# FifthEpoch/longcat-video-tta

Hardware: AMD Instinct MI355X
Metric: denoised latent frames/sec (49x720p, 50-step CFG denoise) (higher is better)
Workload: dtype bf16; 1 GPU; K3: 49x720p (13 latent frames, 46 800 tokens); DiT 48 blocks x 4096 hidden, CFG 4.0, 50-step flow-match Euler, no conditioning frames; depth=48, parallelism=dp1

## Files before the change

### longcat-video-tta_amd/csrc/attn_fwd.hip

```cpp
#include "attn_common.h"
#include <type_traits>

struct AttnFwdParams : AttnFwdLead {
  float scale, scale_log2e;
  int gx, xcd_remap;
};

template <int NWAVES, int PRIO, bool XATTN, int VAR>
__global__ __launch_bounds__(NWAVES * 64) void attn_fwd_kernel(const AttnFwdParams p) {
  constexpr bool DMA = (VAR & 1) != 0;
  constexpr bool UNIT = (VAR & 2) != 0;
  static_assert(!DMA || NWAVES == 8, "LDS-DMA staging is laid out for 8 waves (2 K + 2 V instructions per wave)");
  constexpr int NT = NWAVES * 64;
  constexpr int QROWS = NWAVES * 32;
  constexpr int NCH = 1024 / NT;
  constexpr int TILE_BYTES = 64 * 256;
  extern __shared__ __attribute__((aligned(16))) unsigned char smem[];
  lds_u8* lds = (lds_u8*)smem;

  const int tid = threadIdx.x;
  const int lane = tid & 63;
  const int wave = __builtin_amdgcn_readfirstlane(tid >> 6);
  const int r = lane & 31, h = lane >> 5;
  int qb, head;
// ... 102 lines not shown
  if (PRIO == 1 && wave >= NWAVES / 2) __builtin_amdgcn_s_setprio(1);
  const int nt = (int)((p.d.Nk + 63) / 64);
  {
    if (DMA) {
      dma_tile(0, 0, std::false_type{});
    } else {
      load_tile(0);
      store_tile(0);
    }
    __syncthreads();
  }

  auto tile_body = [&](const int t, auto buf_c, auto last_c, auto next_full_c) {
    constexpr int buf = decltype(buf_c)::value;
    constexpr bool has_next = !decltype(last_c)::value;
    if (has_next) {
      if (DMA) dma_tile(t + 1, buf ^ 1, next_full_c);
      else load_tile((int64_t)(t + 1) * 64);
    }

    const lds_u8* kb = lds + buf * 2 * TILE_BYTES;
    const lds_u8* vb = kb + TILE_BYTES;

    f32x16 s0, s1;
#pragma unroll
    for (int e = 0; e < 16; ++e) { s0[e] = UNIT ? minit[e] : 0.f; s1[e] = UNIT ? minit[e] : 0.f; }
#pragma unroll
    for (int ks = 0; ks < 8; ++ks) {
      const int co = 16 * ((2 * ks + h) ^ kf);
      const bf16x8 a0 = *reinterpret_cast<const __attribute__((address_space(3))) bf16x8*>(kb + k_row_off + co);
      const bf16x8 a1 = *reinterpret_cast<const __attribute__((address_space(3))) bf16x8*>(kb + 32 * 256 + k_row_off + co);
      s0 = __builtin_amdgcn_mfma_f32_32x32x16_bf16(a0, qf[ks], s0, 0, 0, 0);
      s1 = __builtin_amdgcn_mfma_f32_32x32x16_bf16(a1, qf[ks], s1, 0, 0, 0);
    }

    if (!has_next && (p.d.Nk & 63)) {
      const int valid = (int)(p.d.Nk - (int64_t)t * 64);
#pragma unroll
      for (int e = 0; e < 16; ++e) {
        const int key = (e & 3) + 8 * (e >> 2) + 4 * h;
        if (key >= valid) s0[e] = -INFINITY;
        if (key + 32 >= valid) s1[e] = -INFINITY;
      }
    }

    float mxa = s0[0], mxb = s1[0];
#pragma unroll
    for (int e = 1; e < 16; ++e) {
      mxa = fmaxf(mxa, s0[e]);
      mxb = fmaxf(mxb, s1[e]);
    }
    float mx = fmaxf(mxa, mxb);
    mx = half_max(mx);
    float psum = 0.f;
    if constexpr (UNIT) {
      if (__builtin_amdgcn_ballot_w64(mx > ATTN_RESCALE_THR) != 0ull || t == 0) {
        const float d = (t == 0) ? mx : fmaxf(mx, 0.f);
        const float alpha = __builtin_amdgcn_exp2f(-d);
        m_run += d;
        l_run *= alpha;
#pragma unroll
        for (int dd = 0; dd < 4; ++dd)
#pragma unroll
          for (int e = 0; e < 16; ++e) oacc[dd][e] *= alpha;
#pragma unroll
        for (int e = 0; e < 16; ++e) {
          s0[e] -= d;
          s1[e] -= d;
          minit[e] = -m_run;
        }
      }
#pragma unroll
      for (int e = 0; e < 16; ++e) {
        s0[e] = __builtin_amdgcn_exp2f(s0[e]);
        s1[e] = __builtin_amdgcn_exp2f(s1[e]);
        psum += s0[e] + s1[e];
      }
    } else {
      if (__builtin_amdgcn_ballot_w64((mx - m_run) * p.scale_log2e > ATTN_RESCALE_THR) != 0ull) {
        const float m_new = fmaxf(m_run, mx);
        const float alpha = __builtin_amdgcn_exp2f((m_run - m_new) * p.scale_log2e);
        m_run = m_new;
        l_run *= alpha;
#pragma unroll
        for (int d = 0; d < 4; ++d)
#pragma unroll
          for (int e = 0; e < 16; ++e) oacc[d][e] *= alpha;
      }
      const float mc = m_run * p.scale_log2e;
#pragma unroll
      for (int e = 0; e < 16; ++e) {
        s0[e] = __builtin_amdgcn_exp2f(s0[e] * p.scale_log2e - mc);
        s1[e] = __builtin_amdgcn_exp2f(s1[e] * p.scale_log2e - mc);
        psum += s0[e] + s1[e];
      }
    }
    l_run += psum;

    bf16x8 pb[4];
#pragma unroll
    for (int j = 0; j < 8; ++j) {
      pb[0][j] = (__bf16)s0[j];
      pb[1][j] = (__bf16)s0[8 + j];
      pb[2][j] = (__bf16)s1[j];
      pb[3][j] = (__bf16)s1[8 + j];
    }

#pragma unroll
    for (int kk = 0; kk < 4; ++kk) {
#pragma unroll
      for (int d = 0; d < 4; ++d) {
        const int dx = 64 * (d ^ q4);
        const s16x4 lo = __builtin_amdgcn_ds_read_tr16_b64_v4i16(
            (__attribute__((address_space(3))) s16x4*)(vb + v_base[0] + 4096 * kk + dx + 16 * v_low[0]));
        const s16x4 hi = __builtin_amdgcn_ds_read_tr16_b64_v4i16(
            (__attribute__((address_space(3))) s16x4*)(vb + v_base[1] + 4096 * kk + dx + 16 * v_low[1]));
        const bf16x8 vf = __builtin_bit_cast(bf16x8, __builtin_shufflevector(lo, hi, 0, 1, 2, 3, 4, 5, 6, 7));
        oacc[d] = __builtin_amdgcn_mfma_f32_32x32x16_bf16(vf, pb[kk], oacc[d], 0, 0, 0);
      }
    }

    if (has_next && !DMA) store_tile(buf ^ 1);
    __syncthreads();
  };
  {
    using B0 = std::integral_constant<int, 0>;
    using B1 = std::integral_constant<int, 1>;
    using Y = std::true_type;
    using N = std::false_type;
    int t = 0;
    for (; t + 3 < nt; t += 2) {
      tile_body(t, B0{}, N{}, Y{});
      tile_body(t + 1, B1{}, N{}, Y{});
    }
    const int left = nt - t;
    if (left == 3) {
      tile_body(t, B0{}, N{}, Y{});
      tile_body(t + 1, B1{}, N{}, N{});
      tile_body(t + 2, B0{}, Y{}, N{});
    } else if (left == 2) {
      tile_body(t, B0{}, N{}, N{});
      tile_body(t + 1, B1{}, Y{}, N{});
    } else {
      tile_body(t, B0{}, Y{}, N{});
    }
  }

  const float l_tot = half_sum(l_run);
  const float inv = 1.0f / l_tot;
  const int64_t qrow = q0 + r;
  if (qrow < p.d.Nq) {
    bf16_t* op = p.o + b * p.d.o_sb + qrow * p.d.o_sn + (int64_t)head * p.d.o_sh;
#pragma unroll
    for (int d = 0; d < 4; ++d)
#pragma unroll
      for (int i = 0; i < 4; ++i) {
        u16x4 pk;
#pragma unroll
        for (int e = 0; e < 4; ++e) pk[e] = f2bf(oacc[d][4 * i + e] * inv);
        *reinterpret_cast<u16x4*>(op + 32 * d + 8 * i + 4 * h) = pk;
      }
    if (p.lse && h == 0) p.lse[(b * p.d.H + head) * p.d.Nq + qrow] = m_run * p.scale + __logf(l_tot);
  }
}

static thread_local const char* g_last_attn_kernel = "none";
extern "C" const char* lcv_attn_fwd_last_kernel(void) { return g_last_attn_kernel; }

extern "C" int lcv_attn_fwd(const void* q, const void* k, const void* v, void* o, float* lse, int64_t B,
                            int64_t H, int64_t Nq, int64_t Nk, int64_t q_sb, int64_t q_sn, int64_t q_sh,
                            int64_t k_sb, int64_t k_sn, int64_t k_sh, int64_t v_sb, int64_t v_sn,
                            int64_t v_sh, int64_t o_sb, int64_t o_sn, int64_t o_sh, float scale,
                            void* stream) {
  LCV_CHECK_ARG(q && k && v && o, "attn_fwd: null pointer");
  LCV_CHECK_ARG(B > 0 && H > 0 && H <= 65535 && B <= 65535, "attn_fwd: bad B/H");
  LCV_CHECK_ARG(Nk > 0, "attn_fwd: Nk must be > 0 (empty key set has no softmax)");
  LCV_CHECK_ARG(q_sn % 8 == 0 && k_sn % 8 == 0 && v_sn % 8 == 0 && q_sh % 8 == 0 && k_sh % 8 == 0 &&
                    v_sh % 8 == 0 && q_sb % 8 == 0 && k_sb % 8 == 0 && v_sb % 8 == 0,
                "attn_fwd: q/k/v strides must be multiples of 8 elements");
  LCV_CHECK_ARG(o_sn % 4 == 0 && o_sh % 4 == 0 && o_sb % 4 == 0, "attn_fwd: o strides must be multiples of 4 elements");
  LCV_CHECK_ARG(((uintptr_t)q % 16 == 0) && ((uintptr_t)k % 16 == 0) && ((uintptr_t)v % 16 == 0) && ((uintptr_t)o % 8 == 0),
                "attn_fwd: pointers must be 16-byte aligned");
  if (Nq == 0) return LCV_OK;
  AttnArgs a = {};
// ... 38 lines not shown
```

### longcat-video-tta_amd/csrc/elementwise.hip

```cpp
#include "lcv_common.h"
#include "cfg_guidance.h"

#define ROWNORM_MAXCH 8

template <int MODE>
__global__ __launch_bounds__(256) void rownorm_fwd_kernel(
    const bf16_t* __restrict__ x, const float* __restrict__ p_add, const float* __restrict__ p_mul,
    bf16_t* __restrict__ y, int64_t rows, int C, int64_t S, int64_t mod_stride, float eps) {
  const int lane = threadIdx.x & 63;
  const int64_t row = (int64_t)blockIdx.x * 4 + (threadIdx.x >> 6);
  if (row >= rows) return;
  const bf16_t* xr = x + row * C;
  float v[ROWNORM_MAXCH][8];
  float sum = 0.f;
#pragma unroll
  for (int ch = 0; ch < ROWNORM_MAXCH; ++ch) {
    const int c = (ch * 64 + lane) * 8;
    if (c < C) {
      u16x8 raw = *reinterpret_cast<const u16x8*>(xr + c);
      unpack8(raw, v[ch]);
#pragma unroll
      for (int i = 0; i < 8; ++i) sum += v[ch][i];
    } else {
#pragma unroll
// ... 96 lines not shown
}

extern "C" int lcv_gate_residual_fwd(const void* x, const void* y, const float* mod, void* out,
                                     int64_t B, int64_t T, int64_t S, int64_t C, int64_t mod_stride,
                                     int64_t gate_off, void* stream) {
  LCV_CHECK_ARG(x && y && out, "gate_residual_fwd: null pointer");
  LCV_CHECK_ARG(C > 0 && C % 8 == 0, "gate_residual_fwd: C must be a multiple of 8");
  LCV_CHECK_ARG(gate_off % 4 == 0 && mod_stride % 4 == 0, "gate_residual_fwd: offsets must be 16-byte aligned");
  const int64_t n_packets = B * T * S * (C / 8);
  if (n_packets == 0) return LCV_OK;
  int64_t blocks = (n_packets + 255) / 256;
  if (blocks > 256 * 16) blocks = 256 * 16;
  hipLaunchKernelGGL(gate_residual_fwd_kernel, dim3((unsigned)blocks), dim3(256), 0, (hipStream_t)stream,
                     (const bf16_t*)x, (const bf16_t*)y, mod ? mod + gate_off : nullptr, (bf16_t*)out,
                     n_packets, (int)(C / 8), S, mod_stride);
  LCV_LAUNCH_CHECK("gate_residual_fwd");
  return LCV_OK;
}

__device__ __forceinline__ void norm_rope_vec(const bf16_t* src, bf16_t* dst, const float (&w)[8],
                                              const float (&cs)[8], bool do_rope, float eps, float out_scale) {
  float f[8];
  unpack8(*reinterpret_cast<const u16x8*>(src), f);
  float ss = 0.f;
#pragma unroll
  for (int i = 0; i < 8; ++i) ss += f[i] * f[i];
  ss += __shfl_xor(ss, 8, 64);
  ss += __shfl_xor(ss, 4, 64);
  ss += __shfl_xor(ss, 2, 64);
  ss += __shfl_xor(ss, 1, 64);
  const float r = rsqrtf(ss * (1.0f / 128.0f) + eps);
  float o[8];
#pragma unroll
  for (int i = 0; i < 8; ++i) f[i] = bfround(bfround(f[i] * r) * w[i]);
  if (do_rope) {
#pragma unroll
    for (int i = 0; i < 4; ++i) {
      const float c = cs[2 * i], s = cs[2 * i + 1];
      const float x0 = f[2 * i], x1 = f[2 * i + 1];
      o[2 * i] = __fadd_rn(__fmul_rn(x0, c), __fmul_rn(-x1, s));
      o[2 * i + 1] = __fadd_rn(__fmul_rn(x1, c), __fmul_rn(x0, s));
    }
  } else {
#pragma unroll
    for (int i = 0; i < 8; ++i) o[i] = f[i];
  }
#pragma unroll
  for (int i = 0; i < 8; ++i) o[i] *= out_scale;
  *reinterpret_cast<u16x8*>(dst) = pack8(o);
}

__global__ __launch_bounds__(256) void qknorm_rope_fwd_kernel(
    const bf16_t* __restrict__ q_in, const bf16_t* __restrict__ k_in, const bf16_t* __restrict__ v_in,
    bf16_t* __restrict__ q_out, bf16_t* __restrict__ k_out, bf16_t* __restrict__ v_out,
    const bf16_t* __restrict__ wq, const bf16_t* __restrict__ wk, const float* __restrict__ cs_tab,
    int H, int64_t in_sb, int64_t in_sn, int64_t q_sb, int64_t q_sn, int64_t kv_sb, int64_t kv_sn,
    int64_t pos_off, float eps, float q_scale) {
// ... 398 lines not shown
```

### longcat-video-tta_amd/lcv_hip/autograd_ops.py

```python
import weakref
from typing import List, Optional

import torch

from . import ops
from .lib import (LCV_EPI_GELU_TANH, LCV_EPI_NONE, LCV_EPI_SWIGLU, LcvError)

BF16 = torch.bfloat16
F32 = torch.float32

_EPI = {None: LCV_EPI_NONE, "gelu_tanh": LCV_EPI_GELU_TANH}


def _needs_grad(*ts) -> bool:
    return torch.is_grad_enabled() and any(t is not None and t.requires_grad for t in ts)


_WT_CACHE = {}


def transposed_weight(w: torch.Tensor) -> torch.Tensor:
    key = id(w)
    ent = _WT_CACHE.get(key)
    if ent is not None and ent[0]() is w and ent[1] == w._version and ent[2].data_ptr() != 0:
# ... 467 lines not shown
        off = 0
        for b in range(B):
            Lb = int(seqlens[b])
            ops.attention_bwd(qn[b:b + 1], kn[:, off:off + Lb], kv_raw[:, off:off + Lb, 1], o[b:b + 1], do[b:b + 1],
                              lses[b], dqn[b:b + 1], dkv[:, off:off + Lb, 0], dkv[:, off:off + Lb, 1], scale,
                              accumulate_kv=False)
            off += Lb
        dq_raw = torch.empty_like(q_raw)
        dwq = torch.zeros(D, dtype=torch.float32, device=q_raw.device) if want_dw else None
        dwk = torch.zeros(D, dtype=torch.float32, device=q_raw.device) if want_dw else None
        ops.qknorm_rope_bwd(q_raw, None, dqn, None, dq_raw, None, wq, wk, None, 0, eps, dwq=dwq)
        dkv_raw = torch.empty_like(kv_raw)
        ops.qknorm_rope_bwd(None, kv_raw[:, :, 0], None, dkv[:, :, 0], None, dkv_raw[:, :, 0], wq, wk, None, 0, eps, dwk=dwk)
        dkv_raw[:, :, 1].copy_(dkv[:, :, 1])
        return (dq_raw, dkv_raw, dwq.to(wq.dtype) if (want_dw and wq.requires_grad) else None,
                dwk.to(wk.dtype) if (want_dw and wk.requires_grad) else None, None, None, None)


def cross_attention(q, kv, wq, wk, seqlens: List[int], scale, eps):
    if _needs_grad(q, kv, wq, wk):
        return _CrossAttentionFn.apply(q, kv, wq, wk, seqlens, scale, eps)
    B, N, H, D = q.shape
    k, v = kv[:, :, 0], kv[:, :, 1]
    ops.qknorm_rope(q, None, None, q, None, None, wq, wk, None, 0, eps)
    ops.qknorm_rope(None, k, None, None, k, None, wq, wk, None, 0, eps)
    o = torch.empty_like(q)
    off = 0
    for b in range(B):
        Lb = int(seqlens[b])
        ops.attention(q[b:b + 1], k[:, off:off + Lb], v[:, off:off + Lb], scale, out=o[b:b + 1])
        off += Lb
    return o


class _GeluTanhFn(torch.autograd.Function):
    @staticmethod
    def forward(ctx, x):
        ctx.save_for_backward(x)
        return ops.gelu_tanh(x)

    @staticmethod
    def backward(ctx, dy):
        (x,) = ctx.saved_tensors
        return ops.gelu_tanh_bwd(x, (dy if dy.dtype == BF16 else dy.to(BF16)).contiguous())


def gelu_tanh(x: torch.Tensor) -> torch.Tensor:
    if _needs_grad(x):
        return _GeluTanhFn.apply(x)
# ... 105 lines not shown
```

### longcat-video-tta_amd/lcv_hip/build.py

```python
import os
import subprocess
import sys
from concurrent.futures import ThreadPoolExecutor
from pathlib import Path

PKG_DIR = Path(__file__).resolve().parent
CSRC = PKG_DIR.parent / "csrc"
INCLUDE = PKG_DIR.parents[1] / "include"
BUILD = CSRC / "build"
LIB = PKG_DIR / "liblcv_hip.so"
HIPCC = os.environ.get("HIPCC", "/opt/rocm/bin/hipcc")
FLAGS = ["--offload-arch=gfx950", "-O3", "-fPIC", "-std=c++17", "-Wno-unused-value",
         "-fno-gpu-rdc", "-I", str(INCLUDE)]


def _newest_header():
    hs = list(CSRC.glob("*.h")) + list(INCLUDE.glob("*.h"))
    return max(h.stat().st_mtime for h in hs)


_ATTN_FLAGS = ["-fno-honor-nans", "-mno-amdgpu-ieee", "-fno-slp-vectorize"]
EXTRA = {"attn_fwd.hip": _ATTN_FLAGS, "attn_fwd_pipe.hip": _ATTN_FLAGS, "attn_bwd_dq2.hip": _ATTN_FLAGS, "attn_bwd_dkv2.hip": _ATTN_FLAGS,
         "attn_fwd_w64.hip": _ATTN_FLAGS,
         "optim_master.hip": ["-ffp-contract=off"], "optim_moments8.hip": ["-ffp-contract=off"],
         "optim_accum.hip": ["-ffp-contract=off"], "optim_anchor.hip": ["-ffp-contract=off"],
         "optim_ema.hip": ["-ffp-contract=off"], "step_cache.hip": ["-ffp-contract=off"],
         "solver_step.hip": ["-ffp-contract=off"], "cfg_reuse.hip": ["-ffp-contract=off"]}


def _compile(src: Path, hdr_mtime: float) -> Path:
    obj = BUILD / (src.stem + ".o")
    if obj.exists() and obj.stat().st_mtime > max(src.stat().st_mtime, hdr_mtime):
        return obj
    cmd = [HIPCC, *FLAGS, *EXTRA.get(src.name, []), "-c", str(src), "-o", str(obj)]
    r = subprocess.run(cmd, capture_output=True, text=True)
    if r.returncode != 0:
        raise RuntimeError(f"hipcc failed for {src.name}:\n{r.stdout}\n{r.stderr}")
    if r.stderr.strip():
        sys.stderr.write(r.stderr)
    return obj


def build(verbose: bool = False) -> Path:
    BUILD.mkdir(exist_ok=True)
    srcs = sorted(CSRC.glob("*.hip"))
    if not srcs:
# ... 18 lines not shown
```

### longcat-video-tta_amd/lcv_hip/lib.py

```python
import ctypes
import os
from ctypes import c_char_p, c_double, c_float, c_int, c_int64, c_uint64, c_void_p
from pathlib import Path

_LIB_PATH = Path(__file__).resolve().parent / "liblcv_hip.so"

P, I64, F32, I, F64, U64 = c_void_p, c_int64, c_float, c_int, c_double, c_uint64

_SIGNATURES = {
    "lcv_device_check": [],
    "lcv_adaln_modulate_fwd": [P, P, P, I64, I64, I64, I64, I64, I64, I64, F32, P],
    "lcv_adaln_modulate_bwd": [P, P, P, P, P, I64, I64, I64, I64, I64, I64, I64, F32, P, P],
    "lcv_layernorm_affine_fwd": [P, P, P, P, I64, I64, F32, P],
    "lcv_layernorm_affine_bwd": [P, P, P, P, P, P, I64, I64, F32, P, P],
    "lcv_gate_residual_fwd": [P, P, P, P, I64, I64, I64, I64, I64, I64, P],
    "lcv_gate_residual_bwd": [P, P, P, P, P, I64, I64, I64, I64, I64, I64, P],
    "lcv_qknorm_rope_fwd": [P, P, P, P, P, P, P, P, P, I64, I64, I64, I64, I64, I64, I64, I64, I64, I64, F32, F32, P],
    "lcv_qknorm_rope_bwd": [P, P, P, P, P, P, P, P, P, I64, I64, I64, I64, I64, I64, I64, I64, I64, I64, I64, I64, F32, F32, P, P, I64, P],
    "lcv_attn_fwd": [P, P, P, P, P, I64, I64, I64, I64] + [I64] * 12 + [F32, P],
    "lcv_attn_bwd": [P, P, P, P, P, P, P, P, P, P, I, I64, I64, I64, I64] + [I64] * 21 + [F32, P],
    "lcv_gemm_nt": [P, P, P, P, P, P, I64, I64, I64, I64, I64, I64, I64, I64, I64, I, I, P, P, I64, I64, I64, P],
    "lcv_gemm_set_workspace": [P, I64],
    "lcv_linear_f32_smallm": [P, P, P, P, I64, I64, I64, I, P],
    "lcv_lora_down": [P, P, P, I64, I64, I64, I64, I64, F32, P],
# ... 84 lines not shown
}

_SIGNATURES_EMA = {
    "lcv_master_ema_load": [P, P, P, I64, I64, P],
    "lcv_master_ema_update": [P, P, P, I64, I64, F64, P],
    "lcv_master_ema_swap": [P, P, P, I64, I64, P],
}

_SIGNATURES_STEPCACHE = {
    "lcv_stepcache_diff": [P, P, P, P, I64, I64, F32, P, I64, P, P],
    "lcv_stepcache_store": [P, P, P, I64, P],
    "lcv_stepcache_apply": [P, P, P, I64, P],
}

_SIGNATURES_SOLVER = {
    "lcv_cfg_lms_step": [P, P, P, P, P, P, P, I64, I64, F32, F32, F32, F32, I, I, I, P],
}

_SIGNATURES_CFGREUSE = {
    "lcv_cfg_delta_store": [P, P, P, P, P, I64, I64, F32, I, P],
    "lcv_cfg_delta_apply": [P, P, P, I64, I64, P],
}

LCV_EPI_NONE, LCV_EPI_SWIGLU, LCV_EPI_GATE_RESIDUAL, LCV_EPI_GELU_TANH, LCV_EPI_SILU = 0, 1, 2, 3, 4


class LcvError(RuntimeError):
    code = None

    @property
    def fatal(self) -> bool:
        return self.code in (-2, -3)


_lib = None


def lib_path() -> Path:
    return _LIB_PATH


def load():
    global _lib
    if _lib is not None:
        return _lib
    if not _LIB_PATH.exists():
# ... 8 lines not shown
    lib.lcv_last_error.argtypes = []
    lib.lcv_attn_fwd_last_kernel.restype = c_char_p
    lib.lcv_attn_fwd_last_kernel.argtypes = []
    lib.lcv_knobs_list.restype = c_char_p
    lib.lcv_knobs_list.argtypes = []
    lib.lcv_knobs_reload.restype = c_int
    lib.lcv_knobs_reload.argtypes = []
    lib.lcv_conv3d_last_kernel.restype = c_char_p
    lib.lcv_conv3d_last_kernel.argtypes = []
    lib.lcv_tn_skinny_ws_bytes.restype = c_int64
    lib.lcv_tn_skinny_ws_bytes.argtypes = [I64, I64, I64]
    lib.lcv_attn_bwd_ws_floats.restype = c_int64
    lib.lcv_attn_bwd_ws_floats.argtypes = [I64, I64, I64, I64]
    lib.lcv_lpips_ws_bytes.restype = c_int64
    lib.lcv_lpips_ws_bytes.argtypes = [I64, I64, I64]
    lib.lcv_det_ws_bytes.restype = c_int64
    lib.lcv_det_ws_bytes.argtypes = [I, I64, I64, I64]
    lib.lcv_tn_skinny_dropout_ws_bytes.restype = c_int64
    lib.lcv_tn_skinny_dropout_ws_bytes.argtypes = [I64, I64, I64]
    for name, args in (list(_SIGNATURES.items()) + list(_SIGNATURES_LPIPS.items()) + list(_SIGNATURES_DET.items())
                       + list(_SIGNATURES_LORA.items()) + list(_SIGNATURES_MASTER.items()) + list(_SIGNATURES_MOMENTS8.items())
                       + list(_SIGNATURES_ACCUM.items()) + list(_SIGNATURES_ANCHOR.items()) + list(_SIGNATURES_EMA.items())
                       + list(_SIGNATURES_STEPCACHE.items()) + list(_SIGNATURES_SOLVER.items())
                       + list(_SIGNATURES_CFGREUSE.items())):
        fn = getattr(lib, name, None)
        if fn is None:
            continue
        fn.restype = c_int
        fn.argtypes = args
    _lib = lib
    return lib


def reload_knobs() -> int:
    return load().lcv_knobs_reload()


def set_knob(name: str, value) -> None:
    if value is None:
        os.environ.pop(name, None)
    else:
        os.environ[name] = str(value)
    if _lib is not None:
        _lib.lcv_knobs_reload()


def call(name: str, *args):
# ... 9 lines not shown
```

### longcat-video-tta_amd/lcv_hip/ops.py

```python
import os
from typing import Optional, Tuple

import torch

from . import lib as _lib
from .lib import (LCV_EPI_GATE_RESIDUAL, LCV_EPI_GELU_TANH, LCV_EPI_NONE, LCV_EPI_SILU, LCV_EPI_SWIGLU,
                  call)

BF16 = torch.bfloat16
F32 = torch.float32
PROFILE = None
PROFILE_BWD = None


_DETERMINISTIC = os.environ.get("LCV_DETERMINISTIC", "") == "1"


def set_deterministic(flag: bool) -> None:
    global _DETERMINISTIC
    _DETERMINISTIC = bool(flag)


def is_deterministic() -> bool:
    return _DETERMINISTIC
# ... 110 lines not shown

def attention(q: torch.Tensor, k: torch.Tensor, v: torch.Tensor, scale: float,
              out: Optional[torch.Tensor] = None, need_lse: bool = False) -> Tuple[torch.Tensor, Optional[torch.Tensor]]:
    for t, nme in ((q, "q"), (k, "k"), (v, "v")):
        _req(t, BF16, "attention." + nme)
        if t.shape[-1] != 128 or t.stride(-1) != 1:
            raise _lib.LcvError("attention: head_dim must be 128 and contiguous")
    B, Nq, H, D = q.shape
    Nk = k.shape[1]
    if out is None:
        out = torch.empty((B, Nq, H, D), dtype=BF16, device=q.device)
    lse = torch.empty((B, H, Nq), dtype=F32, device=q.device) if need_lse else None
    if PROFILE is not None:
        ev0 = torch.cuda.Event(enable_timing=True); ev1 = torch.cuda.Event(enable_timing=True)
        ev0.record()
    call("lcv_attn_fwd", _ptr(q), _ptr(k), _ptr(v), _ptr(out), _ptr(lse), B, H, Nq, Nk,
         q.stride(0), q.stride(1), q.stride(2), k.stride(0), k.stride(1), k.stride(2),
         v.stride(0), v.stride(1), v.stride(2), out.stride(0), out.stride(1), out.stride(2),
         float(scale), _stream())
    if PROFILE is not None:
        ev1.record()
        PROFILE.append((ev0, ev1, 4.0 * B * H * Nq * Nk * D, Nq, Nk, _lib.load().lcv_attn_fwd_last_kernel().decode()))
    return out, lse


_GEMM_WS = {}
GEMM_WS_BYTES = 256 << 20


def _ensure_gemm_workspace(device: torch.device) -> None:
    idx = device.index if device.index is not None else torch.cuda.current_device()
    if idx not in _GEMM_WS:
        if _GEMM_WS:
            raise _lib.LcvError(
                f"gemm_nt on cuda:{idx}, but this process already bound the library's split-K workspace to cuda:"
                f"{next(iter(_GEMM_WS))}: the build runs one process per GPU (torch.distributed), a second device in the "
                "same process would write its partial sums into the first device's memory")
        ws = torch.empty(GEMM_WS_BYTES, dtype=torch.uint8, device=device)
        call("lcv_gemm_set_workspace", _ptr(ws), GEMM_WS_BYTES)
        _GEMM_WS[idx] = ws


PARAM_EPOCH = 0


def gemm_nt(a: torch.Tensor, w: torch.Tensor, bias: Optional[torch.Tensor] = None, *,
# ... 766 lines not shown
```

Baseline: 0.06241 latent frames/s.

## Add fused text cross-attention kernel with in-kernel Q RMSNorm and resident K/V

Adds a dedicated kernel for cross-attention over short text keys (at most 128 per batch element). It keeps all K/V tiles resident in LDS and fuses the Q RMSNorm into the attention kernel, and each block loops over several query blocks. This replaces a separate qknorm pass over the large video-token Q plus per-batch generic attention launches, cutting one full read and write of Q and the K/V reload per query block. The shared tile math is factored into an include file, and the rsqrt is swapped for a hardware rsq with denormal handling. The cost is a new code path that has to match the numerics of the old one, plus persistent-block scheduling heuristics.

```diff
diff --git a/include/lcv_hip_textattn.h b/include/lcv_hip_textattn.h
--- /dev/null
+++ b/include/lcv_hip_textattn.h
@@ -0,0 +1,21 @@
+#ifndef LCV_HIP_TEXTATTN_H
+#define LCV_HIP_TEXTATTN_H
+
+#include <stdint.h>
+#include "lcv_hip.h"
+
+#ifdef __cplusplus
+extern "C" {
+#endif
+
+#define LCV_TEXT_ATTN_MAX_LEN 128
+#define LCV_TEXT_ATTN_MAX_BATCH 8
+
+int lcv_text_attn_fwd(const void* q, const void* k, const void* v, void* o, const void* wq, const int64_t* seqlens, int64_t B,
+                      int64_t H, int64_t Nq, int64_t q_sb, int64_t q_sn, int64_t q_sh, int64_t kv_sn, int64_t kv_sh,
+                      int64_t o_sb, int64_t o_sn, int64_t o_sh, float scale, float eps, int64_t stretch, void* stream);
+
+#ifdef __cplusplus
+}
+#endif
+#endif
diff --git a/longcat-video-tta_amd/csrc/attn_fwd.hip b/longcat-video-tta_amd/csrc/attn_fwd.hip
--- a/longcat-video-tta_amd/csrc/attn_fwd.hip
+++ b/longcat-video-tta_amd/csrc/attn_fwd.hip
@@ -1,4 +1,5 @@
 #include "attn_common.h"
+#include "attn_tile_math.h"
 #include <type_traits>
 
 struct AttnFwdParams : AttnFwdLead {
@@ -148,103 +149,9 @@
     const lds_u8* kb = lds + buf * 2 * TILE_BYTES;
     const lds_u8* vb = kb + TILE_BYTES;
 
-    f32x16 s0, s1;
-#pragma unroll
-    for (int e = 0; e < 16; ++e) { s0[e] = UNIT ? minit[e] : 0.f; s1[e] = UNIT ? minit[e] : 0.f; }
-#pragma unroll
-    for (int ks = 0; ks < 8; ++ks) {
-      const int co = 16 * ((2 * ks + h) ^ kf);
-      const bf16x8 a0 = *reinterpret_cast<const __attribute__((address_space(3))) bf16x8*>(kb + k_row_off + co);
-      const bf16x8 a1 = *reinterpret_cast<const __attribute__((address_space(3))) bf16x8*>(kb + 32 * 256 + k_row_off + co);
-      s0 = __builtin_amdgcn_mfma_f32_32x32x16_bf16(a0, qf[ks], s0, 0, 0, 0);
-      s1 = __builtin_amdgcn_mfma_f32_32x32x16_bf16(a1, qf[ks], s1, 0, 0, 0);
-    }
-
-    if (!has_next && (p.d.Nk & 63)) {
-      const int valid = (int)(p.d.Nk - (int64_t)t * 64);
-#pragma unroll
-      for (int e = 0; e < 16; ++e) {
-        const int key = (e & 3) + 8 * (e >> 2) + 4 * h;
-        if (key >= valid) s0[e] = -INFINITY;
-        if (key + 32 >= valid) s1[e] = -INFINITY;
-      }
-    }
-
-    float mxa = s0[0], mxb = s1[0];
-#pragma unroll
-    for (int e = 1; e < 16; ++e) {
-      mxa = fmaxf(mxa, s0[e]);
-      mxb = fmaxf(mxb, s1[e]);
-    }
-    float mx = fmaxf(mxa, mxb);
-    mx = half_max(mx);
-    float psum = 0.f;
-    if constexpr (UNIT) {
-      if (__builtin_amdgcn_ballot_w64(mx > ATTN_RESCALE_THR) != 0ull || t == 0) {
-        const float d = (t == 0) ? mx : fmaxf(mx, 0.f);
-        const float alpha = __builtin_amdgcn_exp2f(-d);
-        m_run += d;
-        l_run *= alpha;
-#pragma unroll
-        for (int dd = 0; dd < 4; ++dd)
-#pragma unroll
-          for (int e = 0; e < 16; ++e) oacc[dd][e] *= alpha;
-#pragma unroll
-        for (int e = 0; e < 16; ++e) {
-          s0[e] -= d;
-          s1[e] -= d;
-          minit[e] = -m_run;
-        }
-      }
-#pragma unroll
-      for (int e = 0; e < 16; ++e) {
-        s0[e] = __builtin_amdgcn_exp2f(s0[e]);
-        s1[e] = __builtin_amdgcn_exp2f(s1[e]);
-        psum += s0[e] + s1[e];
-      }
-    } else {
-      if (__builtin_amdgcn_ballot_w64((mx - m_run) * p.scale_log2e > ATTN_RESCALE_THR) != 0ull) {
-        const float m_new = fmaxf(m_run, mx);
-        const float alpha = __builtin_amdgcn_exp2f((m_run - m_new) * p.scale_log2e);
-        m_run = m_new;
-        l_run *= alpha;
-#pragma unroll
-        for (int d = 0; d < 4; ++d)
-#pragma unroll
-          for (int e = 0; e < 16; ++e) oacc[d][e] *= alpha;
-      }
-      const float mc = m_run * p.scale_log2e;
-#pragma unroll
-      for (int e = 0; e < 16; ++e) {
-        s0[e] = __builtin_amdgcn_exp2f(s0[e] * p.scale_log2e - mc);
-        s1[e] = __builtin_amdgcn_exp2f(s1[e] * p.scale_log2e - mc);
-        psum += s0[e] + s1[e];
-      }
-    }
-    l_run += psum;
-
-    bf16x8 pb[4];
-#pragma unroll
-    for (int j = 0; j < 8; ++j) {
-      pb[0][j] = (__bf16)s0[j];
-      pb[1][j] = (__bf16)s0[8 + j];
-      pb[2][j] = (__bf16)s1[j];
-      pb[3][j] = (__bf16)s1[8 + j];
-    }
-
-#pragma unroll
-    for (int kk = 0; kk < 4; ++kk) {
-#pragma unroll
-      for (int d = 0; d < 4; ++d) {
-        const int dx = 64 * (d ^ q4);
-        const s16x4 lo = __builtin_amdgcn_ds_read_tr16_b64_v4i16(
-            (__attribute__((address_space(3))) s16x4*)(vb + v_base[0] + 4096 * kk + dx + 16 * v_low[0]));
-        const s16x4 hi = __builtin_amdgcn_ds_read_tr16_b64_v4i16(
-            (__attribute__((address_space(3))) s16x4*)(vb + v_base[1] + 4096 * kk + dx + 16 * v_low[1]));
-        const bf16x8 vf = __builtin_bit_cast(bf16x8, __builtin_shufflevector(lo, hi, 0, 1, 2, 3, 4, 5, 6, 7));
-        oacc[d] = __builtin_amdgcn_mfma_f32_32x32x16_bf16(vf, pb[kk], oacc[d], 0, 0, 0);
-      }
-    }
+    const int64_t tile_Nk = p.d.Nk;
+    const float tile_scale_log2e = p.scale_log2e;
+#include "attn_tile_math.inc"
 
     if (has_next && !DMA) store_tile(buf ^ 1);
     __syncthreads();
@@ -280,12 +187,8 @@
 #pragma unroll
     for (int d = 0; d < 4; ++d)
 #pragma unroll
-      for (int i = 0; i < 4; ++i) {
-        u16x4 pk;
-#pragma unroll
-        for (int e = 0; e < 4; ++e) pk[e] = f2bf(oacc[d][4 * i + e] * inv);
-        *reinterpret_cast<u16x4*>(op + 32 * d + 8 * i + 4 * h) = pk;
-      }
+      for (int i = 0; i < 4; ++i)
+        *reinterpret_cast<u16x4*>(op + 32 * d + 8 * i + 4 * h) = attn_out_pack(oacc[d], i, inv);
     if (p.lse && h == 0) p.lse[(b * p.d.H + head) * p.d.Nq + qrow] = m_run * p.scale + __logf(l_tot);
   }
 }
diff --git a/longcat-video-tta_amd/csrc/attn_tile_math.h b/longcat-video-tta_amd/csrc/attn_tile_math.h
--- /dev/null
+++ b/longcat-video-tta_amd/csrc/attn_tile_math.h
@@ -0,0 +1,9 @@
+#pragma once
+#include "attn_common.h"
+
+__device__ __forceinline__ u16x4 attn_out_pack(const f32x16& acc, const int i, const float inv) {
+  u16x4 pk;
+#pragma unroll
+  for (int e = 0; e < 4; ++e) pk[e] = f2bf(acc[4 * i + e] * inv);
+  return pk;
+}
diff --git a/longcat-video-tta_amd/csrc/attn_tile_math.inc b/longcat-video-tta_amd/csrc/attn_tile_math.inc
--- /dev/null
+++ b/longcat-video-tta_amd/csrc/attn_tile_math.inc
@@ -0,0 +1,97 @@
+    f32x16 s0, s1;
+  #pragma unroll
+    for (int e = 0; e < 16; ++e) { s0[e] = UNIT ? minit[e] : 0.f; s1[e] = UNIT ? minit[e] : 0.f; }
+  #pragma unroll
+    for (int ks = 0; ks < 8; ++ks) {
+      const int co = 16 * ((2 * ks + h) ^ kf);
+      const bf16x8 a0 = *reinterpret_cast<const __attribute__((address_space(3))) bf16x8*>(kb + k_row_off + co);
+      const bf16x8 a1 = *reinterpret_cast<const __attribute__((address_space(3))) bf16x8*>(kb + 32 * 256 + k_row_off + co);
+      s0 = __builtin_amdgcn_mfma_f32_32x32x16_bf16(a0, qf[ks], s0, 0, 0, 0);
+      s1 = __builtin_amdgcn_mfma_f32_32x32x16_bf16(a1, qf[ks], s1, 0, 0, 0);
+    }
+
+    if (!has_next && (tile_Nk & 63)) {
+      const int valid = (int)(tile_Nk - (int64_t)t * 64);
+  #pragma unroll
+      for (int e = 0; e < 16; ++e) {
+        const int key = (e & 3) + 8 * (e >> 2) + 4 * h;
+        if (key >= valid) s0[e] = -INFINITY;
+        if (key + 32 >= valid) s1[e] = -INFINITY;
+      }
+    }
+
+    float mxa = s0[0], mxb = s1[0];
+  #pragma unroll
+    for (int e = 1; e < 16; ++e) {
+      mxa = fmaxf(mxa, s0[e]);
+      mxb = fmaxf(mxb, s1[e]);
+    }
+    float mx = fmaxf(mxa, mxb);
+    mx = half_max(mx);
+    float psum = 0.f;
+    if constexpr (UNIT) {
+      if (__builtin_amdgcn_ballot_w64(mx > ATTN_RESCALE_THR) != 0ull || t == 0) {
+        const float d = (t == 0) ? mx : fmaxf(mx, 0.f);
+        const float alpha = __builtin_amdgcn_exp2f(-d);
+        m_run += d;
+        l_run *= alpha;
+  #pragma unroll
+        for (int dd = 0; dd < 4; ++dd)
+  #pragma unroll
+          for (int e = 0; e < 16; ++e) oacc[dd][e] *= alpha;
+  #pragma unroll
+        for (int e = 0; e < 16; ++e) {
+          s0[e] -= d;
+          s1[e] -= d;
+          minit[e] = -m_run;
+        }
+      }
+  #pragma unroll
+      for (int e = 0; e < 16; ++e) {
+        s0[e] = __builtin_amdgcn_exp2f(s0[e]);
+        s1[e] = __builtin_amdgcn_exp2f(s1[e]);
+        psum += s0[e] + s1[e];
+      }
+    } else {
+      if (__builtin_amdgcn_ballot_w64((mx - m_run) * tile_scale_log2e > ATTN_RESCALE_THR) != 0ull) {
+        const float m_new = fmaxf(m_run, mx);
+        const float alpha = __builtin_amdgcn_exp2f((m_run - m_new) * tile_scale_log2e);
+        m_run = m_new;
+        l_run *= alpha;
+  #pragma unroll
+        for (int d = 0; d < 4; ++d)
+  #pragma unroll
+          for (int e = 0; e < 16; ++e) oacc[d][e] *= alpha;
+      }
+      const float mc = m_run * tile_scale_log2e;
+  #pragma unroll
+      for (int e = 0; e < 16; ++e) {
+        s0[e] = __builtin_amdgcn_exp2f(s0[e] * tile_scale_log2e - mc);
+        s1[e] = __builtin_amdgcn_exp2f(s1[e] * tile_scale_log2e - mc);
+        psum += s0[e] + s1[e];
+      }
+    }
+    l_run += psum;
+
+    bf16x8 pb[4];
+  #pragma unroll
+    for (int j = 0; j < 8; ++j) {
+      pb[0][j] = (__bf16)s0[j];
+      pb[1][j] = (__bf16)s0[8 + j];
+      pb[2][j] = (__bf16)s1[j];
+      pb[3][j] = (__bf16)s1[8 + j];
+    }
+
+  #pragma unroll
+    for (int kk = 0; kk < 4; ++kk) {
+  #pragma unroll
+      for (int d = 0; d < 4; ++d) {
+        const int dx = 64 * (d ^ q4);
+        const s16x4 lo = __builtin_amdgcn_ds_read_tr16_b64_v4i16(
+            (__attribute__((address_space(3))) s16x4*)(vb + v_base[0] + 4096 * kk + dx + 16 * v_low[0]));
+        const s16x4 hi = __builtin_amdgcn_ds_read_tr16_b64_v4i16(
+            (__attribute__((address_space(3))) s16x4*)(vb + v_base[1] + 4096 * kk + dx + 16 * v_low[1]));
+        const bf16x8 vf = __builtin_bit_cast(bf16x8, __builtin_shufflevector(lo, hi, 0, 1, 2, 3, 4, 5, 6, 7));
+        oacc[d] = __builtin_amdgcn_mfma_f32_32x32x16_bf16(vf, pb[kk], oacc[d], 0, 0, 0);
+      }
+    }
diff --git a/longcat-video-tta_amd/csrc/elementwise.hip b/longcat-video-tta_amd/csrc/elementwise.hip
--- a/longcat-video-tta_amd/csrc/elementwise.hip
+++ b/longcat-video-tta_amd/csrc/elementwise.hip
@@ -1,5 +1,6 @@
 #include "lcv_common.h"
 #include "cfg_guidance.h"
+#include "qk_rmsnorm.h"
 
 #define ROWNORM_MAXCH 8
 
@@ -142,17 +143,14 @@
                                               const float (&cs)[8], bool do_rope, float eps, float out_scale) {
   float f[8];
   unpack8(*reinterpret_cast<const u16x8*>(src), f);
-  float ss = 0.f;
-#pragma unroll
-  for (int i = 0; i < 8; ++i) ss += f[i] * f[i];
+  float ss = qk_rms_slice_ss(f);
   ss += __shfl_xor(ss, 8, 64);
   ss += __shfl_xor(ss, 4, 64);
   ss += __shfl_xor(ss, 2, 64);
   ss += __shfl_xor(ss, 1, 64);
-  const float r = rsqrtf(ss * (1.0f / 128.0f) + eps);
+  const float r = qk_rms_rstd(ss, eps);
   float o[8];
-#pragma unroll
-  for (int i = 0; i < 8; ++i) f[i] = bfround(bfround(f[i] * r) * w[i]);
+  qk_rms_apply(f, r, w);
   if (do_rope) {
 #pragma unroll
     for (int i = 0; i < 4; ++i) {
diff --git a/longcat-video-tta_amd/csrc/qk_rmsnorm.h b/longcat-video-tta_amd/csrc/qk_rmsnorm.h
--- /dev/null
+++ b/longcat-video-tta_amd/csrc/qk_rmsnorm.h
@@ -0,0 +1,23 @@
+#pragma once
+#include "lcv_common.h"
+
+__device__ __forceinline__ float qk_rms_slice_ss(const float (&f)[8]) {
+#pragma clang fp contract(fast)
+  float ss = 0.f;
+#pragma unroll
+  for (int i = 0; i < 8; ++i) ss += f[i] * f[i];
+  return ss;
+}
+
+__device__ __forceinline__ float qk_rms_rstd(float ss, float eps) {
+#pragma clang fp contract(fast)
+  const float x = ss * (1.0f / 128.0f) + eps;
+  const bool tiny = x < 0x1p-126f;
+  const float y = __builtin_amdgcn_rsqf(tiny ? x * 0x1p24f : x);
+  return tiny ? y * 0x1p12f : y;
+}
+
+__device__ __forceinline__ void qk_rms_apply(float (&f)[8], float r, const float (&w)[8]) {
+#pragma unroll
+  for (int i = 0; i < 8; ++i) f[i] = bfround(bfround(f[i] * r) * w[i]);
+}
diff --git a/longcat-video-tta_amd/csrc/text_attn.hip b/longcat-video-tta_amd/csrc/text_attn.hip
--- /dev/null
+++ b/longcat-video-tta_amd/csrc/text_attn.hip
@@ -0,0 +1,232 @@
+#include "attn_common.h"
+#include "attn_tile_math.h"
+#include "qk_rmsnorm.h"
+#include "../../include/lcv_hip_textattn.h"
+#include <type_traits>
+
+struct TextAttnParams : AttnFwdLead {
+  const bf16_t* wq;
+  float scale_log2e, eps;
+  int gx, xcd_remap;
+  int nqb, stretch;
+  int koff[LCV_TEXT_ATTN_MAX_BATCH], klen[LCV_TEXT_ATTN_MAX_BATCH];
+};
+
+#define TEXT_ATTN_WAVES 8
+#define TEXT_ATTN_TILE_BYTES (64 * 256)
+#define TEXT_ATTN_LDS (4 * TEXT_ATTN_TILE_BYTES + TEXT_ATTN_WAVES * 32 * 256 + 256)
+
+__global__ __launch_bounds__(TEXT_ATTN_WAVES * 64) void text_attn_fwd_kernel(const TextAttnParams p) {
+  constexpr bool UNIT = false;
+  constexpr int NT = TEXT_ATTN_WAVES * 64;
+  constexpr int QROWS = TEXT_ATTN_WAVES * 32;
+  constexpr int TILE_BYTES = TEXT_ATTN_TILE_BYTES;
+  extern __shared__ __attribute__((aligned(16))) unsigned char smem[];
+  lds_u8* lds = (lds_u8*)smem;
+
+  const int tid = threadIdx.x;
+  const int lane = tid & 63;
+  const int wave = __builtin_amdgcn_readfirstlane(tid >> 6);
+  const int r = lane & 31, h = lane >> 5;
+  int sb, head;
+  int64_t b;
+  ATTN_BLOCK_DECODE(p, sb, head, b);
+  int L = p.klen[0], koff = p.koff[0];
+#pragma unroll
+  for (int i = 1; i < LCV_TEXT_ATTN_MAX_BATCH; ++i)
+    if (b == i) { L = p.klen[i]; koff = p.koff[i]; }
+  const int nt = (L + 63) >> 6;
+
+  {
+    const bf16_t* kbase = p.k + (int64_t)koff * p.d.k_sn + (int64_t)head * p.d.k_sh;
+    const bf16_t* vbase = p.v + (int64_t)koff * p.d.v_sn + (int64_t)head * p.d.v_sh;
+#pragma unroll
+    for (int i = 0; i < 2 * 1024 / NT; ++i) {
+      const int c = tid + i * NT;
+      const int row = c >> 4, ch = c & 15;
+      if (row < 64 * nt) {
+        const int src = row < L ? row : L - 1;
+        const u32x4 kr = *reinterpret_cast<const u32x4*>(kbase + (int64_t)src * p.d.k_sn + 8 * ch);
+        const u32x4 vr = *reinterpret_cast<const u32x4*>(vbase + (int64_t)src * p.d.v_sn + 8 * ch);
+        lds_u8* dst = lds + (row >> 6) * 2 * TILE_BYTES + attn_tile_off(row & 63, ch);
+        *reinterpret_cast<AS3 u32x4*>(dst) = kr;
+        *reinterpret_cast<AS3 u32x4*>(dst + TILE_BYTES) = vr;
+      }
+    }
+  }
+
+  lds_u8* wlds = lds + 4 * TILE_BYTES + TEXT_ATTN_WAVES * (32 * 256);
+  if (tid < 16) *reinterpret_cast<AS3 u32x4*>(wlds + 16 * tid) = *reinterpret_cast<const u32x4*>(p.wq + 8 * tid);
+
+  lds_u8* stage = lds + 4 * TILE_BYTES + wave * (32 * 256);
+  const int kf = attn_swz(r);
+  const int k_row_off = 256 * r;
+  const int q4 = (lane >> 2) & 3, p4 = lane & 3, g1 = (lane >> 4) & 1;
+  int v_base[2], v_low[2];
+#pragma unroll
+  for (int half = 0; half < 2; ++half) {
+    v_base[half] = 256 * (4 * h + 8 * half + q4) + 8 * (p4 & 1);
+    v_low[half] = (2 * g1 + (p4 >> 1)) ^ (h + 2 * half);
+  }
+  auto lane_again = [&]() { int l = lane; asm volatile("" : "+v"(l)); return l; };
+  const bf16_t* qhead = p.q + b * p.d.q_sb + (int64_t)head * p.d.q_sh;
+  bf16_t* ohead = p.o + b * p.d.o_sb + (int64_t)head * p.d.o_sh;
+  u32x4 pre[8];
+  auto load_q = [&](int qb, int l) {
+    const int64_t q0 = (int64_t)qb * QROWS + wave * 32 + (l >> 4);
+#pragma unroll
+    for (int j = 0; j < 8; ++j) {
+      int64_t row = q0 + 4 * j;
+      if (row > p.d.Nq - 1) row = p.d.Nq - 1;
+      pre[j] = *reinterpret_cast<const u32x4*>(qhead + row * p.d.q_sn + 8 * (l & 15));
+    }
+  };
+
+  const int qb_begin = sb * p.stretch;
+  const int qb_end = qb_begin + p.stretch < p.nqb ? qb_begin + p.stretch : p.nqb;
+  load_q(qb_begin, lane);
+  __syncthreads();
+
+  for (int qb = qb_begin; qb < qb_end; ++qb) {
+    {
+      const int l = lane_again();
+#pragma unroll
+      for (int j = 0; j < 8; ++j) *reinterpret_cast<AS3 u32x4*>(stage + attn_tile_off(4 * j + (l >> 4), l & 15)) = pre[j];
+      __builtin_amdgcn_wave_barrier();
+      if (qb + 1 < qb_end) load_q(qb + 1, l);
+    }
+    u16x8 qraw[8];
+    {
+      const int l = lane_again();
+#pragma unroll
+      for (int ks = 0; ks < 8; ++ks)
+        qraw[ks] = *reinterpret_cast<const AS3 u16x8*>(stage + attn_tile_off(l & 31, 2 * ks + (l >> 5)));
+    }
+
+    bf16x8 qf[8];
+    {
+      float ss[8];
+#pragma unroll
+      for (int ks = 0; ks < 8; ++ks) {
+        float f[8];
+        unpack8(qraw[ks], f);
+        ss[ks] = qk_rms_slice_ss(f);
+      }
+      const float u0 = ss[0] + ss[4], u1 = ss[1] + ss[5], u2 = ss[2] + ss[6], u3 = ss[3] + ss[7];
+      const float v0 = u0 + u2, v1 = u1 + u3;
+      const float rr = qk_rms_rstd(half_sum(v0 + v1), p.eps);
+#pragma unroll
+      for (int ks = 0; ks < 8; ++ks) {
+        float f[8], w[8];
+        unpack8(qraw[ks], f);
+        const u16x8 wv = *reinterpret_cast<const AS3 u16x8*>(wlds + 16 * (2 * ks + h));
+        unpack8(wv, w);
+        qk_rms_apply(f, rr, w);
+        qf[ks] = __builtin_bit_cast(bf16x8, pack8(f));
+      }
+    }
+
+    f32x16 oacc[4];
+#pragma unroll
+    for (int d = 0; d < 4; ++d)
+#pragma unroll
+      for (int e = 0; e < 16; ++e) oacc[d][e] = 0.f;
+    float m_run = -INFINITY;
+    f32x16 minit;
+#pragma unroll
+    for (int e = 0; e < 16; ++e) minit[e] = 0.f;
+    float l_run = 0.f;
+    const int64_t tile_Nk = L;
+    const float tile_scale_log2e = p.scale_log2e;
+    auto tile_body = [&](auto t_c, auto last_c) {
+      constexpr int t = decltype(t_c)::value;
+      constexpr bool has_next = !decltype(last_c)::value;
+      const lds_u8* kb = lds + t * 2 * TILE_BYTES;
+      const lds_u8* vb = kb + TILE_BYTES;
+#include "attn_tile_math.inc"
+    };
+    {
+      using T0 = std::integral_constant<int, 0>;
+      using T1 = std::integral_constant<int, 1>;
+      if (nt == 2) {
+        tile_body(T0{}, std::false_type{});
+        tile_body(T1{}, std::true_type{});
+      } else {
+        tile_body(T0{}, std::true_type{});
+      }
+    }
+
+    const float l_tot = half_sum(l_run);
+    const float inv = 1.0f / l_tot;
+    __builtin_amdgcn_wave_barrier();
+    const int l = lane_again();
+#pragma unroll
+    for (int d = 0; d < 4; ++d)
+#pragma unroll
+      for (int i = 0; i < 4; ++i)
+        *reinterpret_cast<AS3 u16x4*>(stage + attn_tile_off(l & 31, 4 * d + i) + 8 * (l >> 5)) = attn_out_pack(oacc[d], i, inv);
+    __builtin_amdgcn_wave_barrier();
+    const int64_t o0 = (int64_t)qb * QROWS + wave * 32 + (l >> 4);
+#pragma unroll
+    for (int j = 0; j < 8; ++j) {
+      const u32x4 row = *reinterpret_cast<const AS3 u32x4*>(stage + attn_tile_off(4 * j + (l >> 4), l & 15));
+      if (o0 + 4 * j < p.d.Nq) *reinterpret_cast<u32x4*>(ohead + (o0 + 4 * j) * p.d.o_sn + 8 * (l & 15)) = row;
+    }
+    __builtin_amdgcn_wave_barrier();
+  }
+}
+
+extern "C" int lcv_text_attn_fwd(const void* q, const void* k, const void* v, void* o, const void* wq, const int64_t* seqlens,
+                                 int64_t B, int64_t H, int64_t Nq, int64_t q_sb, int64_t q_sn, int64_t q_sh, int64_t kv_sn,
+                                 int64_t kv_sh, int64_t o_sb, int64_t o_sn, int64_t o_sh, float scale, float eps, int64_t stretch,
+                                 void* stream) {
+  LCV_CHECK_ARG(q && k && v && o && wq && seqlens, "text_attn_fwd: null pointer");
+  LCV_CHECK_ARG(B > 0 && B <= LCV_TEXT_ATTN_MAX_BATCH, "text_attn_fwd: B must be 1 .. %d", LCV_TEXT_ATTN_MAX_BATCH);
+  LCV_CHECK_ARG(H > 0 && H <= 65535, "text_attn_fwd: bad H");
+  LCV_CHECK_ARG(Nq >= 0 && Nq < (1ll << 31) - 256 && stretch >= 0, "text_attn_fwd: bad Nq / stretch");
+  LCV_CHECK_ARG(q_sb % 8 == 0 && q_sn % 8 == 0 && q_sh % 8 == 0 && kv_sn % 8 == 0 && kv_sh % 8 == 0 && o_sb % 8 == 0 &&
+                    o_sn % 8 == 0 && o_sh % 8 == 0,
+                "text_attn_fwd: strides must be multiples of 8 elements");
+  LCV_CHECK_ARG(((uintptr_t)q % 16 == 0) && ((uintptr_t)k % 16 == 0) && ((uintptr_t)v % 16 == 0) && ((uintptr_t)o % 16 == 0) &&
+                    ((uintptr_t)wq % 16 == 0),
+                "text_attn_fwd: pointers must be 16-byte aligned");
+  TextAttnParams p = {};
+  int off = 0;
+  for (int64_t b = 0; b < B; ++b) {
+    LCV_CHECK_ARG(seqlens[b] > 0 && seqlens[b] <= LCV_TEXT_ATTN_MAX_LEN, "text_attn_fwd: a text length must be 1 .. %d",
+                  LCV_TEXT_ATTN_MAX_LEN);
+    p.koff[b] = off;
+    p.klen[b] = (int)seqlens[b];
+    off += (int)seqlens[b];
+  }
+  if (Nq == 0) return LCV_OK;
+  p.q = (const bf16_t*)q; p.k = (const bf16_t*)k; p.v = (const bf16_t*)v; p.o = (bf16_t*)o; p.lse = nullptr;
+  p.d.Nq = Nq; p.d.Nk = 0; p.d.H = (int)H;
+  p.d.q_sb = q_sb; p.d.q_sn = q_sn; p.d.q_sh = q_sh;
+  p.d.k_sn = kv_sn; p.d.k_sh = kv_sh; p.d.v_sn = kv_sn; p.d.v_sh = kv_sh;
+  p.d.o_sb = o_sb; p.d.o_sn = o_sn; p.d.o_sh = o_sh;
+  p.wq = (const bf16_t*)wq;
+  p.scale_log2e = scale * 1.4426950408889634f;
+  p.eps = eps;
+  p.nqb = (int)((Nq + TEXT_ATTN_WAVES * 32 - 1) / (TEXT_ATTN_WAVES * 32));
+  if (stretch == 0) {
+    static const int n_cu = [] {
+      int dev = 0, n = 0;
+      if (hipGetDevice(&dev) != hipSuccess || hipDeviceGetAttribute(&n, hipDeviceAttributeMultiprocessorCount, dev) != hipSuccess) n = 0;
+      return n > 0 ? n : 256;
+    }();
+    int64_t per_pair = (2 * (int64_t)n_cu + B * H - 1) / (B * H);
+    if (per_pair < 1) per_pair = 1;
+    stretch = (p.nqb + per_pair - 1) / per_pair;
+  }
+  if (stretch > p.nqb) stretch = p.nqb;
+  p.stretch = (int)stretch;
+  p.gx = (p.nqb + p.stretch - 1) / p.stretch;
+  const char* xe = lcv_knob("LCV_ATTN_XCD");
+  p.xcd_remap = (!(xe && xe[0] == '0') && (B * H) % 8 == 0) ? 1 : 0;
+  const dim3 grid = p.xcd_remap ? dim3((unsigned)p.gx * (unsigned)(H * B)) : dim3((unsigned)p.gx, (unsigned)H, (unsigned)B);
+  ATTN_RAISE_LDS_ONCE("text_attn_fwd", attn_raise_lds((const void*)text_attn_fwd_kernel, TEXT_ATTN_LDS));
+  hipLaunchKernelGGL(text_attn_fwd_kernel, grid, dim3(TEXT_ATTN_WAVES * 64), TEXT_ATTN_LDS, (hipStream_t)stream, p);
+  LCV_LAUNCH_CHECK("text_attn_fwd");
+  return LCV_OK;
+}
diff --git a/longcat-video-tta_amd/lcv_hip/autograd_ops.py b/longcat-video-tta_amd/lcv_hip/autograd_ops.py
--- a/longcat-video-tta_amd/lcv_hip/autograd_ops.py
+++ b/longcat-video-tta_amd/lcv_hip/autograd_ops.py
@@ -1,3 +1,4 @@
+import os
 import weakref
 from typing import List, Optional
 
@@ -513,9 +514,11 @@
         return _CrossAttentionFn.apply(q, kv, wq, wk, seqlens, scale, eps)
     B, N, H, D = q.shape
     k, v = kv[:, :, 0], kv[:, :, 1]
-    ops.qknorm_rope(q, None, None, q, None, None, wq, wk, None, 0, eps)
     ops.qknorm_rope(None, k, None, None, k, None, wq, wk, None, 0, eps)
     o = torch.empty_like(q)
+    if os.environ.get("LCV_TEXT_ATTN", "1") != "0" and ops.text_attention_fits(B, seqlens):
+        return ops.text_attention(q, k, v, wq, seqlens, scale, eps, out=o)
+    ops.qknorm_rope(q, None, None, q, None, None, wq, wk, None, 0, eps)
     off = 0
     for b in range(B):
         Lb = int(seqlens[b])
diff --git a/longcat-video-tta_amd/lcv_hip/build.py b/longcat-video-tta_amd/lcv_hip/build.py
--- a/longcat-video-tta_amd/lcv_hip/build.py
+++ b/longcat-video-tta_amd/lcv_hip/build.py
@@ -15,13 +15,13 @@
 
 
 def _newest_header():
-    hs = list(CSRC.glob("*.h")) + list(INCLUDE.glob("*.h"))
+    hs = list(CSRC.glob("*.h")) + list(CSRC.glob("*.inc")) + list(INCLUDE.glob("*.h"))
     return max(h.stat().st_mtime for h in hs)
 
 
 _ATTN_FLAGS = ["-fno-honor-nans", "-mno-amdgpu-ieee", "-fno-slp-vectorize"]
 EXTRA = {"attn_fwd.hip": _ATTN_FLAGS, "attn_fwd_pipe.hip": _ATTN_FLAGS, "attn_bwd_dq2.hip": _ATTN_FLAGS, "attn_bwd_dkv2.hip": _ATTN_FLAGS,
-         "attn_fwd_w64.hip": _ATTN_FLAGS,
+         "attn_fwd_w64.hip": _ATTN_FLAGS, "text_attn.hip": _ATTN_FLAGS,
          "optim_master.hip": ["-ffp-contract=off"], "optim_moments8.hip": ["-ffp-contract=off"],
          "optim_accum.hip": ["-ffp-contract=off"], "optim_anchor.hip": ["-ffp-contract=off"],
          "optim_ema.hip": ["-ffp-contract=off"], "step_cache.hip": ["-ffp-contract=off"],
diff --git a/longcat-video-tta_amd/lcv_hip/lib.py b/longcat-video-tta_amd/lcv_hip/lib.py
--- a/longcat-video-tta_amd/lcv_hip/lib.py
+++ b/longcat-video-tta_amd/lcv_hip/lib.py
@@ -130,6 +130,11 @@
     "lcv_cfg_delta_apply": [P, P, P, I64, I64, P],
 }
 
+_SIGNATURES_TEXTATTN = {
+    "lcv_text_attn_fwd": [P, P, P, P, P, P, I64, I64, I64] + [I64] * 8 + [F32, F32, I64, P],
+}
+LCV_TEXT_ATTN_MAX_LEN, LCV_TEXT_ATTN_MAX_BATCH = 128, 8
+
 LCV_EPI_NONE, LCV_EPI_SWIGLU, LCV_EPI_GATE_RESIDUAL, LCV_EPI_GELU_TANH, LCV_EPI_SILU = 0, 1, 2, 3, 4
 
 
@@ -184,7 +189,7 @@
                        + list(_SIGNATURES_LORA.items()) + list(_SIGNATURES_MASTER.items()) + list(_SIGNATURES_MOMENTS8.items())
                        + list(_SIGNATURES_ACCUM.items()) + list(_SIGNATURES_ANCHOR.items()) + list(_SIGNATURES_EMA.items())
                        + list(_SIGNATURES_STEPCACHE.items()) + list(_SIGNATURES_SOLVER.items())
-                       + list(_SIGNATURES_CFGREUSE.items())):
+                       + list(_SIGNATURES_CFGREUSE.items()) + list(_SIGNATURES_TEXTATTN.items())):
         fn = getattr(lib, name, None)
         if fn is None:
             continue
diff --git a/longcat-video-tta_amd/lcv_hip/ops.py b/longcat-video-tta_amd/lcv_hip/ops.py
--- a/longcat-video-tta_amd/lcv_hip/ops.py
+++ b/longcat-video-tta_amd/lcv_hip/ops.py
@@ -156,6 +156,40 @@
         ev1.record()
         PROFILE.append((ev0, ev1, 4.0 * B * H * Nq * Nk * D, Nq, Nk, _lib.load().lcv_attn_fwd_last_kernel().decode()))
     return out, lse
+
+
+def text_attention_fits(B: int, seqlens) -> bool:
+    return 1 <= B <= _lib.LCV_TEXT_ATTN_MAX_BATCH and all(1 <= int(n) <= _lib.LCV_TEXT_ATTN_MAX_LEN for n in seqlens)
+
+
+def text_attention(q: torch.Tensor, k: torch.Tensor, v: torch.Tensor, wq: torch.Tensor, seqlens, scale: float,
+                   eps: float = 1e-6, out: Optional[torch.Tensor] = None, stretch: int = 0) -> torch.Tensor:
+    for t, nme in ((q, "q"), (k, "k"), (v, "v"), (wq, "wq")):
+        _req(t, BF16, "text_attention." + nme)
+    B, Nq, H, D = q.shape
+    seqlens = [int(n) for n in seqlens]
+    if D != 128 or k.shape[-1] != 128 or any(t.stride(-1) != 1 for t in (q, k, v)):
+        raise _lib.LcvError("text_attention: head_dim must be 128 and contiguous")
+    if len(seqlens) != B or k.shape[0] != 1 or v.shape != k.shape or k.shape[1] != sum(seqlens) or k.shape[2] != H:
+        raise _lib.LcvError("text_attention: k / v must be [1, sum(seqlens), H, 128] with one length per batch element")
+    if k.stride(1) != v.stride(1) or k.stride(2) != v.stride(2):
+        raise _lib.LcvError("text_attention: k and v must share strides")
+    if not text_attention_fits(B, seqlens):
+        raise _lib.LcvError("text_attention: batch or a text length beyond the resident cap (ask text_attention_fits first)")
+    wq = wq.contiguous()
+    if out is None:
+        out = torch.empty((B, Nq, H, D), dtype=BF16, device=q.device)
+    lens = (_lib.c_int64 * B)(*seqlens)
+    if PROFILE is not None:
+        ev0 = torch.cuda.Event(enable_timing=True); ev1 = torch.cuda.Event(enable_timing=True)
+        ev0.record()
+    call("lcv_text_attn_fwd", _ptr(q), _ptr(k), _ptr(v), _ptr(out), _ptr(wq), lens, B, H, Nq,
+         q.stride(0), q.stride(1), q.stride(2), k.stride(1), k.stride(2), out.stride(0), out.stride(1), out.stride(2),
+         float(scale), float(eps), int(stretch), _stream())
+    if PROFILE is not None:
+        ev1.record()
+        PROFILE.append((ev0, ev1, 4.0 * Nq * sum(seqlens) * H * D, Nq, max(seqlens), "text_attn_fwd_kernel"))
+    return out
 
 
 _GEMM_WS = {}
```

New measurement: 0.06276 latent frames/s (median of 6 runs). No clear change (+0.6%).
